# meilisearch/arroy

Measured on AMD Instinct MI355X. Metric: distances/sec, Q=1 batched 768-dim cosine scan (GB/s vs HBM roofline in `roofline`); tree-build seconds at 10M vectors in `build_10m`, higher is better.
Workload: dtype f32; 1 GPU; 1M x 768 cosine Q=1 scan (configs[1])

## Files before the change

arroy_amd/csrc/common.h:

```cpp
#pragma once

#include <hip/hip_runtime.h>

#include <algorithm>
#include <cstdarg>
#include <cstdint>
#include <cstdio>
#include <atomic>
#include <cstring>
#include <mutex>
#include <new>
#include <string>
#include <thread>
#include <vector>

#include "../../include/arroy_hip.h"
#include "../../include/arroy_hip_policy.h"

namespace ah {

void set_error(const char *fmt, ...);
const char *last_error();
void set_error_status(int status);
void set_error_detail(uint32_t item, uint64_t expected, uint64_t received);
// ... 102 lines not shown
    X(PAIR_GROUP, "AH_PAIR_GROUP", 0)                                                                                    \
    X(PAIR_RUNS, "AH_PAIR_RUNS", 1)                                                                                      \
    X(SEARCH_BITMAP, "AH_SEARCH_BITMAP", 1)          \
    X(SEARCH_TILES, "AH_SEARCH_TILES", 1)                          \
    X(SEARCH_WAVE, "AH_SEARCH_WAVE", 1)                        \
    X(SEARCH_BLOCK_MAX_QUERIES, "AH_SEARCH_BLOCK_MAX_QUERIES", 64)  \
    X(SEARCH_SMALL_GATE, "AH_SEARCH_SMALL_GATE", 1)  \
    X(SEARCH_SMALL_UNITS_MAX_QUERIES, "AH_SEARCH_SMALL_UNITS_MAX_QUERIES", 64)  \
    X(SEARCH_FUSED_FLAG, "AH_SEARCH_FUSED_FLAG", 1)  \
    X(SEARCH_FUSED_PREPARE, "AH_SEARCH_FUSED_PREPARE", 1)  \
    X(SEARCH_SINGLE_FUSED, "AH_SEARCH_SINGLE_FUSED", 1)  \
    X(SEARCH_SMALL_TILES_MAX_QUERIES, "AH_SEARCH_SMALL_TILES_MAX_QUERIES", 8)  \
    X(SEARCH_MULTI, "AH_SEARCH_MULTI", 1)        \
    X(SEARCH_MULTI_TREES_PER_BLOCK, "AH_SEARCH_MULTI_TREES_PER_BLOCK", 8)  \
    X(SEARCH_MULTI_IDS_BY_TILES, "AH_SEARCH_MULTI_IDS_BY_TILES", 1)  \
    X(SEARCH_SPIN_WAIT, "AH_SEARCH_SPIN_WAIT", 1)  \
    X(SEARCH_FLAT_TILES, "AH_SEARCH_FLAT_TILES", 1)  \
    X(SEARCH_STATUS_WIPE, "AH_SEARCH_STATUS_WIPE", 1)  \
    X(SEARCH_ITEM_LIST, "AH_SEARCH_ITEM_LIST", 1)  \
    X(SEARCH_MULTI_OWN_UNITS, "AH_SEARCH_MULTI_OWN_UNITS", 1)  \
    X(SEARCH_MULTI_TRACE, "AH_SEARCH_MULTI_TRACE", 0)  \
    X(SEARCH_MULTI_MAX_QUERIES, "AH_SEARCH_MULTI_MAX_QUERIES", 32)  \
    X(EXACT_WIDE, "AH_EXACT_WIDE", 1)            \
    X(RERANK_GROUPS, "AH_RERANK_GROUPS", 2)      \
    X(RERANK_SCREEN8, "AH_RERANK_SCREEN8", 1)    \
    X(SEARCH_SCREEN8_MAX_VISITS, "AH_SEARCH_SCREEN8_MAX_VISITS", 4)  \
    X(SEARCH_SCREEN8_MIN_QUERIES, "AH_SEARCH_SCREEN8_MIN_QUERIES", 65)  \
    X(SEARCH_SCREEN8, "AH_SEARCH_SCREEN8", 1)    \
    X(RERANK_SCREEN, "AH_RERANK_SCREEN", 1)      \
    X(REPLICATE_HOST_BOUNCE, "AH_REPLICATE_HOST_BOUNCE", 0)  \
    X(RERANK_TIMING, "AH_RERANK_TIMING", 0)      \
    X(SEARCH_SCREEN, "AH_SEARCH_SCREEN", 1)      \
    X(SEARCH_FILTER_GROUP_MIN, "AH_SEARCH_FILTER_GROUP_MIN", 16)  \
    X(FILTER_COMBINE_SHORTCUT, "AH_FILTER_COMBINE_SHORTCUT", 1)  \
    X(AUDIT_COVER_MB, "AH_AUDIT_COVER_MB", 64)  \
    X(HOST_THREADS, "AH_HOST_THREADS", 8)             \
    X(DEVICE_CACHE_MB, "AH_DEVICE_CACHE_MB", 98304)  \
    X(HOST_CACHE_MB, "AH_HOST_CACHE_MB", 16384)    \
    X(CACHE_KEEP_IDLE, "AH_CACHE_KEEP_IDLE", 0)  \
    X(FAIL_ALLOC_AFTER, "AH_FAIL_ALLOC_AFTER", 0)  \
    X(STAGE_THREADS, "AH_STAGE_THREADS", 0)                                                                              \
    X(STAGE_MEMCPY, "AH_STAGE_MEMCPY", 0)                                                                                \
    X(STAGE_REGISTER, "AH_STAGE_REGISTER", 0)
enum Tunable {
#define AH_X(id, name, def) TUN_##id,
    AH_TUNABLES(AH_X)
// ... 340 lines not shown
```

arroy_amd/csrc/dense_device.h:

```cpp
#pragma once

namespace ah {

typedef _Float16 f16x8_t __attribute__((ext_vector_type(8)));
typedef float f32x16_t __attribute__((ext_vector_type(16)));
typedef float f32x4_t __attribute__((ext_vector_type(4)));

constexpr uint32_t kDM = 256;
template <int WN>
struct DenseShape {
    static constexpr uint32_t kBN = 64u * WN;
    static constexpr uint32_t kThreads = 128u * WN;
    static constexpr uint32_t kWaves = 2u * WN;
    static constexpr uint32_t kStage = (kDM + kBN) * 128u;
    static constexpr uint32_t kPiecesA = 32u / kWaves, kPiecesB = (kBN / 8u) / kWaves;
};
constexpr uint32_t kDenseHalf = 128;
constexpr uint32_t kDensePitch = kDM + 4;
constexpr uint32_t kDenseLds = kDenseHalf * kDensePitch * 4;
constexpr uint32_t kDenseGroup = 8;
static_assert(2 * DenseShape<4>::kStage <= kDenseLds && 2 * DenseShape<2>::kStage <= kDenseLds, "stage buffers fit");

constexpr uint32_t kSideUndecided = 2u;
constexpr uint32_t kSideVerify = 4u;

struct DenseArgs {
    const uint16_t *rows;
    const float4 *stats;
    const float *headers;
    uint64_t n;
    uint32_t hpitch;
    const uint8_t *shadow;
    uint64_t hstride;
    uint32_t n_cols;
    const FNode *nodes;
    const uint32_t *node_of;
    uint8_t *side_bytes;
    float gamma_s, gamma_r;
    uint32_t n_row_tiles, n_col_tiles, group, verify;
};

template <int WN>
__device__ __forceinline__ void dense_stage(const uint8_t *const (&a_src)[DenseShape<WN>::kPiecesA],
                                            const uint8_t *const (&b_src)[DenseShape<WN>::kPiecesB], uint32_t kb, uint8_t *stage,
                                            uint32_t wave) {
    typedef DenseShape<WN> SH;
    const uint64_t koff = (uint64_t)kb * 128u;
// ... 450 lines not shown
```

arroy_amd/csrc/forest.hip:

```cpp
#include <algorithm>
#include <atomic>
#include <chrono>
#include <condition_variable>
#include <deque>
#include <thread>
#include <cstdlib>
#include <immintrin.h>
#include <sys/mman.h>
#include <sys/syscall.h>
#include <unistd.h>
#include <new>

#include "common.h"
#include "split_device.h"
#include "screen_device.h"

namespace ah {

static constexpr uint32_t kTile = 2048;
static constexpr int kBlock = 256;
static constexpr int kMaxBlocks = 4096;

enum { ST_PENDING = 0, ST_ACCEPTED = 1, ST_RANDOM = 2 };

// ... 1044 lines not shown
        if (threadIdx.x == 0) {
            tile_left[tile] = s_left;
            if (s_left) atomicAdd(&nodes[tl.node].n_left, s_left);
        }
    }
    __syncthreads();
    if (threadIdx.x == 0) s_fb = s_bad = s_n8 = s_d8 = s_d8b = 0;
    __syncthreads();
    if (j == 0 && fallbacks) atomicAdd(&s_fb, fallbacks);
    if (j == 0 && bad) atomicAdd(&s_bad, bad);
    if (j == 0 && met8) atomicAdd(&s_n8, met8);
    if (j == 0 && decided8) atomicAdd(&s_d8, decided8);
    if (j == 0 && decided8b) atomicAdd(&s_d8b, decided8b);
    __syncthreads();
    if (threadIdx.x == 0) {
        if (s_fb) atomicAdd(&counters->fallbacks, (unsigned long long)s_fb);
        if (s_bad) atomicAdd(&counters->violations, (unsigned long long)s_bad);
        if (s_n8) atomicAdd(&counters->stage8_pairs, (unsigned long long)s_n8);
        if (s_d8) atomicAdd(&counters->stage8_decided, (unsigned long long)s_d8);
        if (s_d8b) atomicAdd(&counters->stage8b_decided, (unsigned long long)s_d8b);
    }
}

template <int METRIC>
__device__ __forceinline__ float rows_exact_margin(const DataView &dv, uint64_t row, const uint8_t *nrec, uint64_t hdr_off,
                                                   uint32_t j) {
    const float *rp = dv.rows_f32 + row * dv.pitch;
    const float *np = reinterpret_cast<const float *>(nrec);
    const float d = octet_reduce_stream<OP_DOT>(reinterpret_cast<const float4 *>(np), rp, dv.dims, j);
    const float *nh = reinterpret_cast<const float *>(nrec + hdr_off);
    if (METRIC == AH_EUCLIDEAN || METRIC == AH_MANHATTAN) return f_add(nh[0], d);
    if (METRIC == AH_DOT_PRODUCT) return f_add(d, f_mul(nh[0], dv.headers[2 * row]));
    return d;
}

template <int METRIC>
__device__ __forceinline__ float rows_exact_margin_wide(const DataView &dv, uint64_t row, const uint8_t *nrec, uint64_t hdr_off,
                                                        uint32_t j) {
    const float *rp = dv.rows_f32 + row * dv.pitch;
    const float *np = reinterpret_cast<const float *>(nrec);
    const float *nh = reinterpret_cast<const float *>(nrec + hdr_off);
    float h0 = 0.0f, rh = 0.0f;
    if (METRIC == AH_EUCLIDEAN || METRIC == AH_MANHATTAN || METRIC == AH_DOT_PRODUCT) h0 = nh[0];
    if (METRIC == AH_DOT_PRODUCT) rh = dv.headers[2 * row];
    const float d = octet_reduce_wide<OP_DOT, false>(np, rp, dv.dims, j);
    if (METRIC == AH_EUCLIDEAN || METRIC == AH_MANHATTAN) return f_add(h0, d);
// ... 50 lines not shown
        const uint32_t rem = slot % per_chunk;
        tile = rem % sch.tiles;
        group = ((x + 8u - (chunk & 7u)) & 7u) + 8u * (rem / sch.tiles);
        if (group >= sch.n_groups) return false;
    } else {
        const uint32_t per_chunk = sch.n_groups * sch.tiles;
        chunk = sch.chunk0 + b / per_chunk;
        const uint32_t in_chunk = b % per_chunk;
        group = in_chunk / sch.tiles;
        tile = in_chunk % sch.tiles;
    }
    row_begin = (uint64_t)chunk * sch.chunk_rows + (uint64_t)tile * sch.rows_per_block;
    row_end = min(min(row_begin + sch.rows_per_block, (uint64_t)(chunk + 1) * sch.chunk_rows), n_rows);
    return row_begin < row_end;
}
__global__ void k_rows_schedule_coverage(RowsSchedule sch, uint64_t n_rows, uint32_t *__restrict__ counts) {
    uint32_t group;
    uint64_t row_begin, row_end;
    if (!rows_block_map(sch, blockIdx.x, n_rows, group, row_begin, row_end)) return;
    for (uint64_t row = row_begin + (threadIdx.x >> 3); row < row_end; row += blockDim.x >> 3)
        if ((threadIdx.x & 7u) == 0) atomicAdd(&counts[(uint64_t)group * n_rows + row], 1u);
}

template <int METRIC, int TC, bool LDS_NORMALS>
__global__ __launch_bounds__(LDS_NORMALS ? (TC >= 16 ? 512 : 1024) : kBlock,
                             LDS_NORMALS ? 1 : (AH_SCREEN_WAVES > 1 ? AH_SCREEN_WAVES : (TC == 8 ? 4 : 1))) void k_forest_screen_rows(
    DataView dv, ScreenView sv, const uint32_t *__restrict__ node_of, uint32_t tree_base, uint32_t n_pass,
    const uint8_t *__restrict__ normals, uint64_t nstride, uint64_t hdr_off, const uint8_t *__restrict__ shadow,
    uint64_t hstride, uint8_t *__restrict__ side_bytes, RowsSchedule sch, const AbortFlags abort_flag,
    ScreenCounters *__restrict__ counters, uint32_t verify) {
    extern __shared__ uint4 s_shadow4[];
    __shared__ uint32_t s_fb, s_bad;
    if (abort_requested(abort_flag)) return;
    uint32_t group;
    uint64_t row_begin, row_end;
    if (!rows_block_map(sch, blockIdx.x, dv.n, group, row_begin, row_end)) return;
    const uint32_t tree0 = tree_base + group * TC;
    const uint32_t hstride4 = (uint32_t)(hstride >> 4);
    uint32_t first_node = 0;
    if (LDS_NORMALS) {
        first_node = sch.tree_first[tree0];
        const uint32_t n_group_nodes = sch.tree_first[tree0 + n_pass] - first_node;
        const uint4 *g = reinterpret_cast<const uint4 *>(shadow + (uint64_t)first_node * hstride);
        const uint32_t total = n_group_nodes * hstride4;
        for (uint32_t i = threadIdx.x; i < total; i += blockDim.x) s_shadow4[i] = g[i];
    }
    if (threadIdx.x == 0) s_fb = s_bad = 0;
    __syncthreads();
    const uint32_t j = threadIdx.x & 7u;
    const uint32_t octets = blockDim.x >> 3;
    const uint32_t steps = sv.hpitch >> 6;
    const uint32_t stats4 = sv.hpitch >> 3;
    const uint4 *base4 = LDS_NORMALS ? s_shadow4 : reinterpret_cast<const uint4 *>(shadow);
    const uint32_t node0 = first_node;
    const uint32_t last_tree = n_pass - 1;
    constexpr int N = TC >= 8 ? 8 : TC;
    constexpr int SETS = TC >= 8 ? TC / 8 : 1;
    const uint32_t my_t = octet_owned_tree<N>(j);
    const bool owner = octet_is_owner<N>(j);
    uint32_t fallbacks = 0, bad = 0;
    for (uint64_t row = row_begin + (threadIdx.x >> 3); row < row_end; row += octets) {
        const uint4 *r4 = reinterpret_cast<const uint4 *>(sv.rows + row * sv.hpitch) + j;
        uint32_t my_node[SETS];
        uint32_t noff[TC];
        float acc[TC];
#pragma unroll
        for (int st = 0; st < SETS; st++)
            my_node[st] = node_of[(uint64_t)(tree0 + min(my_t + 8u * st, last_tree)) * dv.n + row];
#pragma unroll
        for (int t = 0; t < TC; t++) {
// ... 13 lines not shown
        for (; k < steps; k++) {
            const uint4 x = r4[k * 8];
#pragma unroll
            for (int t = 0; t < TC; t++) acc[t] = screen_dot8(base4[noff[t] + k * 8], x, acc[t]);
        }
        const float4 rs = sv.stats[row];
        const float row_extra = METRIC == AH_DOT_PRODUCT ? dv.headers[2 * row] : 0.0f;
#pragma unroll
        for (int st = 0; st < SETS; st++) {
            const float total = octet_transpose_sum<N>(acc + 8 * st, j);
            const uint32_t t = my_t + 8u * st;
            const bool valid = owner && t <= last_tree && my_node[st] != 0xFFFFFFFFu;
            uint32_t side = 0;
            bool decided = false;
            if (valid) {
                const uint4 raw = base4[(my_node[st] - node0) * hstride4 + stats4];
                NormalStats ns;
                ns.an = __uint_as_float(raw.x);
                ns.bn = __uint_as_float(raw.y);
                ns.cn = __uint_as_float(raw.z);
                ns.extra = __uint_as_float(raw.w);
                decided = screen_decides<METRIC>(total, rs, ns, row_extra, sv.gamma_s, sv.gamma_r, side);
            }
            const unsigned long long und = __ballot(valid && (!decided || verify));
            const uint32_t mask8 = (uint32_t)(und >> (8u * ((threadIdx.x & 63u) >> 3))) & 0xFFu;
            if (mask8) {
#pragma unroll
                for (int tt = 0; tt < N; tt++) {
                    constexpr uint32_t kOwner[8] = {octet_owner_lane<N>(0), octet_owner_lane<N>(1), octet_owner_lane<N>(2),
                                                    octet_owner_lane<N>(3), octet_owner_lane<N>(4), octet_owner_lane<N>(5),
                                                    octet_owner_lane<N>(6), octet_owner_lane<N>(7)};
                    const uint32_t ol = kOwner[tt];
                    if ((mask8 >> ol) & 1u) {
                        const uint32_t node = (noff[8 * st + tt] - j) / hstride4 + node0;
                        const uint32_t exact =
                            side_of_margin(rows_exact_margin<METRIC>(dv, row, normals + (uint64_t)node * nstride, hdr_off, j));
                        if (j == ol) {
                            if (decided && exact != side) bad++;
                            if (!decided) fallbacks++;
                            side = exact;
                        }
                    }
                }
            }
            if (valid) side_bytes[(uint64_t)(tree0 + t) * dv.n + row] = (uint8_t)side;
        }
    }
    if (fallbacks) atomicAdd(&s_fb, fallbacks);
    if (bad) atomicAdd(&s_bad, bad);
    __syncthreads();
    if (threadIdx.x == 0) {
        if (s_fb) atomicAdd(&counters->fallbacks, (unsigned long long)s_fb);
        if (s_bad) atomicAdd(&counters->violations, (unsigned long long)s_bad);
    }
}

struct NextCounts {
    uint32_t kids, tiles;
};
__device__ __forceinline__ void child_counts(const FNode &nd, uint32_t split_after, uint32_t cnt[2], uint32_t split[2]) {
    cnt[0] = nd.n_left;
    cnt[1] = nd.count - nd.n_left;
    split[0] = cnt[0] > split_after ? 1u : 0u;
    split[1] = cnt[1] > split_after ? 1u : 0u;
}
__global__ __launch_bounds__(256) void k_next_count(const FNode *__restrict__ nodes, uint32_t n_nodes, uint32_t split_after,
                                                    NextCounts *__restrict__ block_sums) {
    __shared__ uint32_t s_k[4], s_t[4];
    const uint32_t i = blockIdx.x * 256 + threadIdx.x;
    uint32_t kids = 0, tiles = 0;
// ... 421 lines not shown
        AH_HIP(create_copy_stream(&side));
        return AH_OK;
    }
    ~BatchCleanup() {
        if (side) (void)hipStreamSynchronize(side);
        for (hipEvent_t e : ev_attempt)
            if (e) (void)hipEventDestroy(e);
        for (hipEvent_t e : {ev_begin, ev_end, ev_level, ev_copy[0], ev_copy[1]})
            if (e) (void)hipEventDestroy(e);
        if (side) (void)hipStreamDestroy(side);
    }
};

struct CostPt {
    double mb, ns;
};
template <size_t N>
double interp(const CostPt (&t)[N], double mb) {
    if (mb <= t[0].mb) return t[0].ns;
    for (size_t i = 1; i < N; i++)
        if (mb <= t[i].mb) return t[i - 1].ns + (t[i].ns - t[i - 1].ns) * (mb - t[i - 1].mb) / (t[i].mb - t[i - 1].mb);
    return t[N - 1].ns;
}
double rows_pass_ns_per_row(uint32_t tc, double ws_mb, bool screened) {
    static const CostPt e16[] = {{0.4, 1.60}, {3.2, 1.83}, {6.3, 2.05}, {12.6, 2.33}, {25, 5.08}, {50, 6.05}, {100, 6.5}, {400, 6.8}};
    static const CostPt e8[] = {{0.2, 1.16}, {1.6, 1.22}, {3.2, 2.0}, {6.3, 2.5}, {12.6, 3.1}, {25, 3.5}, {100, 3.7}};
    static const CostPt e4[] = {{0.1, 0.73}, {0.8, 0.85}, {3.2, 0.88}, {6.3, 1.07}, {12.6, 1.45}, {25, 1.85}, {50, 2.05}, {100, 2.14}};
    static const CostPt e2[] = {{0.05, 0.49}, {0.8, 0.60}, {3.1, 0.62}, {6.3, 0.74}, {12.6, 0.99}, {25, 1.14}, {50, 1.21}};
    static const CostPt s16[] = {{0.025, 1.11}, {0.2, 1.13}, {0.4, 1.20}, {0.8, 1.25}, {1.6, 1.30}, {3.2, 1.45}, {6.4, 1.99},
                                 {12.7, 2.94}, {25, 3.57}, {51, 3.92}, {102, 4.10}, {203, 4.21}};
    static const CostPt s8[] = {{0.012, 0.58}, {0.1, 0.61}, {0.2, 0.67}, {0.4, 0.71}, {0.8, 0.74}, {1.6, 0.77}, {3.2, 0.85},
                                {6.4, 1.24}, {12.7, 1.66}, {25, 1.94}, {51, 2.09}, {102, 2.15}};
    static const CostPt s4[] = {{0.025, 0.325}, {0.05, 0.353}, {0.1, 0.415}, {0.2, 0.463}, {0.4, 0.493}, {0.8, 0.511},
                                {1.7, 0.45}, {3.4, 0.50}, {6.8, 0.69}, {13.6, 0.90}, {27, 1.03}, {54, 1.10}};
    static const CostPt s2[] = {{0.003, 0.235}, {0.05, 0.243}, {0.1, 0.261}, {0.2, 0.274}, {0.4, 0.284}, {0.8, 0.292},
                                {1.6, 0.314}, {3.2, 0.389}, {6.4, 0.49}, {12.7, 0.56}, {25, 0.60}};
    if (screened) return tc >= 16 ? interp(s16, ws_mb) : tc == 8 ? interp(s8, ws_mb) : tc == 4 ? interp(s4, ws_mb) : interp(s2, ws_mb);
    return tc >= 16 ? interp(e16, ws_mb) : tc == 8 ? interp(e8, ws_mb) : tc == 4 ? interp(e4, ws_mb) : interp(e2, ws_mb);
}

enum { MM_NODE = 0, MM_ROWS2 = 1, MM_ROWS4 = 2, MM_ROWS8 = 3, MM_ROWS16 = 4, MM_LDS8 = 5, MM_LDS16 = 6, MM_BQ = 7 };
inline int mm_rows(uint32_t tc) { return tc >= 16 ? MM_ROWS16 : tc == 8 ? MM_ROWS8 : tc == 4 ? MM_ROWS4 : MM_ROWS2; }

}

static size_t records_pool_trim() {
    RecordsPool &pool = records_pool();
    std::vector<HostRec> r;
    std::vector<uint32_t> i;
    {
        std::lock_guard<std::mutex> lk(pool.mu);
        r.swap(pool.recs);
        i.swap(pool.index);
    }
    return r.capacity() * sizeof(HostRec) + i.capacity() * sizeof(uint32_t);
}
static uint64_t normal_record_stride(const ah_dataset *ds) {
    const uint64_t raw = ds->row_bytes() + 16;
    return metric_is_bq(ds->metric) ? raw : (raw + 127) & ~(uint64_t)127;
// ... 381 lines not shown
            std::lock_guard<std::mutex> lk(mu);
            stop = true;
        }
        cv.notify_all();
        th.join();
    }
};

namespace {
struct ScreenRowsArgs {
    DataView dv;
    ScreenView sv;
    const uint32_t *node_of;
    uint32_t tree_base, n_pass;
    const uint8_t *normals;
    uint64_t nstride, hdr_off;
    const uint8_t *shadow;
    uint64_t hstride;
    uint8_t *side_bytes;
    RowsSchedule sch;
    AbortFlags abort_flag;
    ScreenCounters *counters;
    uint32_t verify;
};
template <int M, int TC, bool LDS>
int launch_screen_rows_inst(const ScreenRowsArgs &a, unsigned grid, size_t sh, hipStream_t s, int device) {
    const unsigned threads = LDS ? (TC >= 16 ? 512u : 1024u) : (unsigned)kBlock;
    if (LDS) {
        static std::atomic<bool> opt_in[64];
        if (!opt_in[device & 63].load(std::memory_order_acquire)) {
            AH_HIP(hipFuncSetAttribute(reinterpret_cast<const void *>(k_forest_screen_rows<M, TC, LDS>),
                                       hipFuncAttributeMaxDynamicSharedMemorySize, (int)kLdsNormalsBytes));
            opt_in[device & 63].store(true, std::memory_order_release);
        }
    }
    hipLaunchKernelGGL((k_forest_screen_rows<M, TC, LDS>), dim3(grid), dim3(threads), LDS ? sh : 0, s, a.dv, a.sv, a.node_of,
                       a.tree_base, a.n_pass, a.normals, a.nstride, a.hdr_off, a.shadow, a.hstride, a.side_bytes, a.sch,
                       a.abort_flag, a.counters, a.verify);
    return AH_OK;
}
template <int M>
int launch_screen_rows_metric(uint32_t tc, bool lds, const ScreenRowsArgs &a, unsigned grid, size_t sh, hipStream_t s, int device) {
    if (lds) return tc >= 16 ? launch_screen_rows_inst<M, 16, true>(a, grid, sh, s, device)
                             : launch_screen_rows_inst<M, 8, true>(a, grid, sh, s, device);
    switch (tc) {
    case 16: return launch_screen_rows_inst<M, 16, false>(a, grid, sh, s, device);
    case 8: return launch_screen_rows_inst<M, 8, false>(a, grid, sh, s, device);
    case 4: return launch_screen_rows_inst<M, 4, false>(a, grid, sh, s, device);
    default: return launch_screen_rows_inst<M, 2, false>(a, grid, sh, s, device);
    }
}
int launch_screen_rows(int metric, uint32_t tc, bool lds, const ScreenRowsArgs &a, unsigned grid, size_t sh, hipStream_t s,
                       int device) {
    switch (metric) {
    case AH_EUCLIDEAN: return launch_screen_rows_metric<AH_EUCLIDEAN>(tc, lds, a, grid, sh, s, device);
    case AH_MANHATTAN: return launch_screen_rows_metric<AH_MANHATTAN>(tc, lds, a, grid, sh, s, device);
    case AH_COSINE: return launch_screen_rows_metric<AH_COSINE>(tc, lds, a, grid, sh, s, device);
    default: return launch_screen_rows_metric<AH_DOT_PRODUCT>(tc, lds, a, grid, sh, s, device);
    }
}
}

namespace {
struct DensePlan {
    uint32_t n_row_tiles, n_col_tiles, group;
    bool wide;
    int narrow;
    bool stream;
    uint32_t tile_rows, tile_cols, threads, lds;
    uint64_t grid;
};
DensePlan dense_plan(uint64_t N, uint32_t n_cols) {
    DensePlan p{};
// ... 81 lines not shown
};

static int build_batch(ah_dataset *ds, const ah_build_options *opt, uint32_t first_tree, uint32_t n_trees,
                       uint32_t split_after, ah_forest *forest, Context *ctx, const uint32_t *subset_ids,
                       const uint64_t *subset_offsets, StreamBuild *sb = nullptr) {
    const uint64_t N = ds->n;
    const auto t_batch = std::chrono::steady_clock::now();
    std::vector<uint64_t> tree_base(n_trees + 1, 0);
    for (uint32_t t = 0; t < n_trees; t++)
        tree_base[t + 1] = tree_base[t] + (subset_ids ? subset_offsets[first_tree + t + 1] - subset_offsets[first_tree + t] : N);
    const uint64_t M = tree_base[n_trees];
    const DataView dv = ds->view();
    hipStream_t s = ctx->stream;
    const bool bq = metric_is_bq(ds->metric);
    const uint64_t hdr_off = ds->row_bytes();
    const uint64_t nstride = normal_record_stride(ds);
    const bool g_screen = tun(TUN_SCREEN) != 0, g_screen_verify = tun(TUN_SCREEN_VERIFY) != 0;
    const int g_rows_force = (int)tun(TUN_ROWMAJOR), g_dense = (int)tun(TUN_DENSE);
    const uint32_t g_tile_blocks = (uint32_t)std::max<long long>(1, tun(TUN_FOREST_TILE_BLOCKS));
    const uint32_t g_node_blocks = (uint32_t)std::max<long long>(0, tun(TUN_FOREST_NODE_BLOCKS));
    const uint32_t g_split_blocks = (uint32_t)std::max<long long>(1, tun(TUN_FOREST_SPLIT_BLOCKS));
    const uint32_t g_row_blocks = (uint32_t)std::max<long long>(1, tun(TUN_FOREST_ROW_BLOCKS));
    const bool g_rows_advance = tun(TUN_ROWMAJOR_ADVANCE) != 0, g_rows_lds = tun(TUN_ROWMAJOR_LDS) != 0;
    const uint32_t g_rows_max_tc = (uint32_t)std::max<long long>(2, tun(TUN_ROWMAJOR_MAX_TC));
    const double g_rows_cache_mb = (double)tun(TUN_ROWMAJOR_CACHE_MB);
    const uint32_t g_dense_max_cols = (uint32_t)std::max<long long>(0, tun(TUN_DENSE_MAX_COLS));
    const double g_dense_gmacs = (double)std::max<long long>(1, tun(TUN_DENSE_GMACS));
    const int timing = (int)tun(TUN_TIMING);
    const bool g_retry_gate = tun(TUN_RETRY_GATE) != 0;
    const uint32_t env_mode = (uint32_t)tun(TUN_MARGIN_MODE) & 0xFFFu;
    const uint32_t mode_req = (opt->margin_mode & 0xFFFu) ? (opt->margin_mode & 0xFFFu) : env_mode;
    const bool exact_only = (opt->margin_mode & AH_MARGIN_EXACT_ONLY) != 0 || !g_screen;

    const uint64_t max_nodes = M / ((uint64_t)split_after + 1) + n_trees;
    const uint64_t max_tiles = M / kTile + n_trees + max_nodes;
    DevBuf<uint32_t> perm_a, perm_b, final_perm, tile_left, tile_left_off, d_child, d_small;
    DevBuf<FNode> d_nodes_a, d_nodes_b, d_nodes_c;
    DevBuf<GroupInfo> d_groups;
    DevBuf<FTile> d_tiles;
    DevBuf<uint64_t> masks;
    DevBuf<NextCounts> d_block_sums;
    AH_TRY(perm_a.ensure(M));
    AH_TRY(perm_b.ensure(M));
    AH_TRY(final_perm.ensure(M));
    AH_TRY(d_nodes_a.ensure(max_nodes));
    AH_TRY(d_nodes_b.ensure(max_nodes));
// ... 612 lines not shown
                                                 : std::min<uint32_t>(n_tiles, std::max<uint32_t>(2048u, std::min<uint32_t>(65536u, n_tiles / 16u)));
        const unsigned masks_grid = n_nodes <= 4 * n_trees ? std::min<uint32_t>(tile_grid, 32768u) : tile_grid;

        const uint64_t rec_bytes = screen ? hstride : nstride;
        const uint64_t nodes_per_tree = (n_nodes + n_trees - 1) / n_trees;
        uint32_t row_tc = 0, lds_tc = 0, lds_worst = 0;
        double best_cost = -1.0;
        if (grouped) {
        } else if (rows_allowed && mode_req == AH_MARGIN_AUTO) {
            const double scale = screen ? (double)ds->hpitch * 2 / 1536.0 : (double)ds->row_bytes() / 3072.0;
            const double node8_ns = sv.rows8_lo ? std::min(0.24, 0.135 + 0.15 * ds->screen8_quality)
                                                : std::min(0.24, 0.155 + 0.125 * ds->screen8_quality);
            const double node_ns = screen ? (screen8 && ds->metric != AH_DOT_PRODUCT ? node8_ns : 0.24) : 0.47;
            const double active = (double)info.pairs / ((double)n_trees * (double)N);
            const double cost_node = (double)info.pairs * node_ns * scale;
            const double convert = (double)n_trees * (double)N *
                                   ((prev_rows && g_rows_advance ? 0.007 : 0.01 + 0.03 * std::min(1.0, (double)nodes_per_tree / 256.0)) +
                                    0.012 * std::min(1.0, (double)nodes_per_tree / 512.0));
            double best = 0.97 * cost_node;
            const double floor_ns = screen ? 0.15 : 0.45;
            auto launch_ns_per_row = [&](uint32_t tcv, uint32_t groups) {
                double ws_mb = (double)((uint64_t)tcv * nodes_per_tree * rec_bytes) / 1e6;
                if (groups <= 2 && tcv >= 16) ws_mb *= 0.5;
                return groups * (floor_ns + (rows_pass_ns_per_row(tcv, ws_mb, screen) - floor_ns) * std::min(1.0, active * 1.05));
            };
            for (uint32_t tc = std::min(16u, g_rows_max_tc); tc >= 2; tc >>= 1) {
                if (tc > 2 && tc / 2 >= n_trees) continue;
                const double ws_mb = (double)((uint64_t)tc * nodes_per_tree * rec_bytes) / 1e6;
                if (g_rows_cache_mb > 0 && ws_mb > g_rows_cache_mb) continue;
                double ns_per_row = n_trees / tc ? launch_ns_per_row(tc, n_trees / tc) : 0.0;
                for (uint32_t t0 = n_trees / tc * tc; t0 < n_trees;) {
                    const uint32_t rem = n_trees - t0;
                    uint32_t tcv = tc;
                    while (tcv > 2 && tcv > rem) tcv >>= 1;
                    for (uint32_t up = tcv << 1; up <= tc && tcv < rem; up <<= 1)
                        if (up >= rem && up - rem <= (up >= 16 ? 3u : 1u)) tcv = up;
                    ns_per_row += launch_ns_per_row(tcv, 1);
                    t0 += std::min(tcv, rem);
                }
                const double cost_rows = (double)N * ns_per_row * scale + convert;
                if (cost_rows < best || (g_rows_force == 1 && row_tc == 0)) {
                    best = std::min(best, cost_rows);
                    row_tc = tc;
                }
            }
            best_cost = best;
        } else if (rows_allowed && mode_req != AH_MARGIN_DENSE_MFMA) {
            row_tc = mode_req & 0xFFu;
        }
        bool dense = false;
        const DensePlan dp_legal = dense_plan(N, std::max(n_nodes, 1u));
        const bool dense_legal = !grouped && rows_allowed && screen && g_dense != 0 && n_nodes <= g_dense_max_cols &&
                                 (dp_legal.grid + 64) * (uint64_t)dp_legal.threads < 0xFFFFFFFFull && dp_legal.grid < 0x7FFFFFFFull;
        if (dense_legal && mode_req == AH_MARGIN_DENSE_MFMA) {
            dense = true;
        } else if (dense_legal && mode_req == AH_MARGIN_AUTO) {
            const uint32_t bn = n_nodes > 128 ? 256u : 128u;
            const double cols = (double)(((uint64_t)n_nodes + bn - 1) / bn * bn);
            const double hscale = (double)ds->hpitch / 768.0;
            const double per_row = std::max(std::max(0.40 * hscale, 0.25), 0.17 * hscale + 0.0023 * n_trees + cols * (double)ds->hpitch / g_dense_gmacs);
            const double convert = (double)n_trees * (double)N * (prev_rows && g_rows_advance ? 0.007 : 0.04);
            const double cost_dense = (double)N * per_row + (double)info.pairs * (0.002 + 0.006 * (double)ds->row_bytes() / 3072.0) + convert;
            dense = g_dense == 1 || best_cost < 0 || cost_dense < best_cost;
// ... 56 lines not shown
            AH_SPLIT_KERNEL(AH_SPLIT_LAUNCH)
#undef AH_SPLIT_LAUNCH
            AH_DBG(s, "create_split");
            if (screen)
                hipLaunchKernelGGL(k_forest_shadow_normals, dim3(std::min<uint32_t>(n_nodes, attempt ? 65536u : 1u << 20)), dim3(64), 0, s,
                                   dv, d_cur, chunk_d, nstride, hdr_off, shadow_d, hstride, sv.hpitch, n_nodes, gate);
            if (screen8 && !(attempt == 0 && row_tc >= 2))
                hipLaunchKernelGGL(k_forest_shadow_normals8, dim3(std::min<uint32_t>(n_nodes, 65536u)), dim3(64), 0, s, dv, d_cur,
                                   n_nodes, chunk_d, nstride, hdr_off, ds->d_dim_scale, shadow8_d, stride8, sv.pitch8, gate);
            AH_HIP(hipEventRecord(bc.ev_attempt[2 * attempt], s));
            if (attempt == 0 && row_tc >= 2) {
                if (prev_rows && g_rows_advance) {
                    hipLaunchKernelGGL(k_forest_advance_node_of, dim3(kMaxBlocks), dim3(kBlock), 0, s, node_of.p, side_bytes.p,
                                       d_child.p, (uint64_t)n_trees * N);
                    if (info.n_fix)
                        hipLaunchKernelGGL(k_forest_assign_node_of, dim3(std::min<uint32_t>(n_tiles, kMaxBlocks)), dim3(kBlock), 0,
                                           s, d_cur, d_tiles.p, n_tiles, cur, N, node_of.p, 1u);
                } else {
                    AH_HIP(hipMemsetAsync(node_of.p, 0xFF, (size_t)n_trees * N * 4, s));
                    hipLaunchKernelGGL(k_forest_assign_node_of, dim3(tile_grid), dim3(kBlock), 0, s, d_cur, d_tiles.p, n_tiles,
                                       cur, N, node_of.p, 0u);
                }
                uint32_t passes = 0;
                if (dense) {
                    DenseArgs da{};
                    da.rows = sv.rows;
                    da.stats = sv.stats;
                    da.headers = dv.headers;
                    da.n = N;
                    da.hpitch = sv.hpitch;
                    da.shadow = shadow_d;
                    da.hstride = hstride;
                    da.n_cols = n_nodes;
                    da.nodes = d_cur;
                    da.node_of = node_of.p;
                    da.side_bytes = side_bytes.p;
                    da.gamma_s = (float)(2.0 * ((double)sv.hpitch + (double)sv.hpitch / 16 + 16.0) * 1.1920929e-7);
                    da.gamma_r = sv.gamma_r;
                    const DensePlan dp = dense_plan(N, n_nodes);
                    da.n_row_tiles = dp.n_row_tiles;
                    da.n_col_tiles = dp.n_col_tiles;
                    da.group = dp.group;
                    da.verify = verify;
                    const bool wide = dp.wide;
                    const uint64_t dgrid = dp.grid;
                    AH_REQUIRE(dgrid < 0x7FFFFFFFull, AH_ERR_INVALID_ARGUMENT, "forest build: too many tiles for one launch");
                    const unsigned egrid = exact_pairs_grid(N, n_trees);
#define AH_DENSE_WN(M, WNV)                                                                                              \
    do {                                                                                                                 \
        static std::atomic<bool> dense_opt_in[64];                               \
        if (!dense_opt_in[ds->device & 63].load(std::memory_order_acquire)) {                                            \
            AH_HIP(hipFuncSetAttribute(reinterpret_cast<const void *>(k_forest_dense_screen<M, WNV>),                    \
                                       hipFuncAttributeMaxDynamicSharedMemorySize, (int)kDenseLds));                     \
            dense_opt_in[ds->device & 63].store(true, std::memory_order_release);                                        \
        }                                                                                                                \
        hipLaunchKernelGGL((k_forest_dense_screen<M, WNV>), dim3((unsigned)dgrid), dim3(DenseShape<WNV>::kThreads),      \
                           kDenseLds, s, da, d_abort);                                                                   \
    } while (0)
#define AH_DENSE_NARROW(M, NTV)                                                                                          \
    do {                                                                                                                 \
        if (dp.stream)                                                                                                   \
            hipLaunchKernelGGL((k_forest_dense_narrow<M, NTV, true>), dim3((unsigned)dgrid), dim3(kNarrowThreads),       \
                               NarrowShape<NTV>::kLds, s, da, d_abort);                                                  \
        else                                                                                                             \
            hipLaunchKernelGGL((k_forest_dense_narrow<M, NTV, false>), dim3((unsigned)dgrid), dim3(kNarrowThreads),      \
                               NarrowShape<NTV>::kLds, s, da, d_abort);                                                  \
    } while (0)
#define AH_DENSE(M)                                                                                                      \
    do {                                                                                                                 \
        if (dp.narrow == 2) AH_DENSE_NARROW(M, 2);                                                                       \
        else if (dp.narrow == 4) AH_DENSE_NARROW(M, 4);                                                                  \
        else if (wide) AH_DENSE_WN(M, 4);                                                                                \
        else AH_DENSE_WN(M, 2);                                                                                          \
        if (tun(TUN_EXACT_WIDE) != 0)                                                                                    \
            hipLaunchKernelGGL((k_forest_exact_pairs<M, true>), dim3(egrid), dim3(256), 0, s, dv, node_of.p, side_bytes.p, \
                               n_trees, chunk_d, nstride, hdr_off, d_counters, d_abort);                                 \
        else                                                                                                             \
            hipLaunchKernelGGL((k_forest_exact_pairs<M>), dim3(egrid), dim3(256), 0, s, dv, node_of.p, side_bytes.p,     \
                               n_trees, chunk_d, nstride, hdr_off, d_counters, d_abort);                                 \
    } while (0)
                    switch (ds->metric) {
                    case AH_EUCLIDEAN: AH_DENSE(AH_EUCLIDEAN); break;
                    case AH_MANHATTAN: AH_DENSE(AH_MANHATTAN); break;
                    case AH_COSINE: AH_DENSE(AH_COSINE); break;
                    default: AH_DENSE(AH_DOT_PRODUCT); break;
                    }
#undef AH_DENSE_WN
#undef AH_DENSE_NARROW
#undef AH_DENSE
                    forest->stats.dense_launches++;
                    forest->stats.dense_columns += n_nodes;
                    passes = 1;
                } else if (screen) {
                    const uint32_t gtc = lds_tc ? lds_tc : row_tc;
                    ScreenRowsArgs ra{dv, sv, node_of.p, 0, 0, chunk_d, nstride, hdr_off, shadow_d, hstride, side_bytes.p,
                                      RowsSchedule{}, d_abort, d_counters, verify};
                    if (lds_tc) {
                        memcpy(h_tree_first, tree_first.data(), ((size_t)n_trees + 1) * 4);
                        AH_HIP(hipMemcpyAsync(d_tree_first_fixed, h_tree_first, ((size_t)n_trees + 1) * 4, hipMemcpyHostToDevice, s));
                    }
                    const size_t lds_sh = (size_t)lds_worst * rec_bytes;
                    auto launch = [&](uint32_t tcv, uint32_t t0, uint32_t groups, uint32_t np) -> int {
                        RowsPlan plan;
                        AH_TRY(plan_rows_launches(N, sv.hpitch, tcv, groups, lds_tc != 0, (uint64_t)tcv * nodes_per_tree * rec_bytes, &plan));
                        ra.tree_base = t0;
                        ra.n_pass = np;
                        ra.sch = plan.sch;
                        ra.sch.tree_first = d_tree_first_fixed;
                        for (const auto &l : plan.launches) {
                            ra.sch.chunk0 = l.first;
                            AH_TRY(launch_screen_rows(ds->metric, tcv, lds_tc != 0, ra, l.second, lds_sh, s, ds->device));
                        }
                        forest->stats.margin_mode_launches[lds_tc ? (tcv >= 16 ? MM_LDS16 : MM_LDS8) : mm_rows(tcv)]++;
                        forest->stats.rows_xcd_launches += plan.xcd ? plan.launches.size() : 0;
                        forest->stats.rows_nt_launches += plan.nt ? plan.launches.size() : 0;
                        forest->stats.rows_split_launches += plan.launches.size() - 1;
                        passes += groups;
                        return AH_OK;
                    };
                    const uint32_t full = n_trees / gtc;
                    if (full) AH_TRY(launch(gtc, 0, full, gtc));
                    for (uint32_t t0 = full * gtc; t0 < n_trees;) {
                        const uint32_t rem = n_trees - t0;
                        uint32_t tcv = gtc;
                        if (!lds_tc) {
                            while (tcv > 2 && tcv > rem) tcv >>= 1;
                            for (uint32_t up = tcv << 1; up <= gtc && tcv < rem; up <<= 1)
                                if (up >= rem && up - rem <= (up >= 16 ? 3u : 1u)) tcv = up;
                        }
                        const uint32_t np = std::min<uint32_t>(tcv, rem);
                        AH_TRY(launch(tcv, t0, 1, np));
                        t0 += np;
                    }
                }
                const unsigned row_grid = (unsigned)std::min<uint64_t>((N + 31) / 32, g_row_blocks);
                for (uint32_t t0 = 0; t0 < n_trees && lds_tc && !screen; t0 += lds_tc) {
                    const uint32_t np = std::min<uint32_t>(lds_tc, n_trees - t0);
                    const uint32_t first = tree_first[t0], cnt = tree_first[t0 + np] - first;
                    if (cnt == 0) continue;
                    const size_t sh = (size_t)cnt * rec_bytes;
                    const unsigned per_cu = (unsigned)std::max<size_t>(1, std::min<size_t>(2, (150u << 10) / std::max<size_t>(sh, 1)));
                    const unsigned lthreads = lds_tc >= 16 ? 512u : 1024u;
                    const unsigned lgrid = (unsigned)std::min<uint64_t>((N * 8 + lthreads - 1) / lthreads, 256u * per_cu);
#define AH_LDS_OPT_IN(KERNEL)                                                                                          \
    do {                                                                                                               \
        static std::atomic<bool> lds_opt_in[64];                                \
        if (!lds_opt_in[ds->device & 63].load(std::memory_order_acquire)) {                                            \
            AH_HIP(hipFuncSetAttribute(reinterpret_cast<const void *>(KERNEL), hipFuncAttributeMaxDynamicSharedMemorySize, \
                                       (int)kLdsNormalsBytes));                                                        \
            lds_opt_in[ds->device & 63].store(true, std::memory_order_release);                                        \
        }                                                                                                              \
    } while (0)
#define AH_ROWS_LDS(M, TCV)                                                                                              \
    do {                                                                                                                 \
        AH_LDS_OPT_IN((k_forest_margin_rows_lds<M, TCV>));                                                               \
        hipLaunchKernelGGL((k_forest_margin_rows_lds<M, TCV>), dim3(lgrid), dim3(lthreads), sh, s, dv, node_of.p, t0, np,  \
// ... 857 lines not shown
```

Measured before the change: 3.051 billion distances/s.

## Defer exact margin fallbacks in screened row kernel to separate exact-pairs pass

The screened row-major forest kernel gains a DEFER variant that only writes undecided/verify markers into side bytes and skips the inline exact-dot fallback. A separate k_forest_exact_pairs launch, shared with the dense path, then resolves those pairs. The goal is to stop divergent per-octet exact work from stalling the screening loop. The cost model gets new deferred-pass tables plus an exact-pairs cost term, so the tree-count choice can shift, and there is one extra kernel launch.

```diff
diff --git a/arroy_amd/csrc/common.h b/arroy_amd/csrc/common.h
--- a/arroy_amd/csrc/common.h
+++ b/arroy_amd/csrc/common.h
@@ -148,6 +148,7 @@
     X(SEARCH_MULTI_TRACE, "AH_SEARCH_MULTI_TRACE", 0)  \
     X(SEARCH_MULTI_MAX_QUERIES, "AH_SEARCH_MULTI_MAX_QUERIES", 32)  \
     X(EXACT_WIDE, "AH_EXACT_WIDE", 1)            \
+    X(ROWS_DEFER_EXACT, "AH_ROWS_DEFER_EXACT", 1)  \
     X(RERANK_GROUPS, "AH_RERANK_GROUPS", 2)      \
     X(RERANK_SCREEN8, "AH_RERANK_SCREEN8", 1)    \
     X(SEARCH_SCREEN8_MAX_VISITS, "AH_SEARCH_SCREEN8_MAX_VISITS", 4)  \
diff --git a/arroy_amd/csrc/dense_device.h b/arroy_amd/csrc/dense_device.h
--- a/arroy_amd/csrc/dense_device.h
+++ b/arroy_amd/csrc/dense_device.h
@@ -21,8 +21,6 @@
 constexpr uint32_t kDenseGroup = 8;
 static_assert(2 * DenseShape<4>::kStage <= kDenseLds && 2 * DenseShape<2>::kStage <= kDenseLds, "stage buffers fit");
 
-constexpr uint32_t kSideUndecided = 2u;
-constexpr uint32_t kSideVerify = 4u;
 
 struct DenseArgs {
     const uint16_t *rows;
diff --git a/arroy_amd/csrc/forest.hip b/arroy_amd/csrc/forest.hip
--- a/arroy_amd/csrc/forest.hip
+++ b/arroy_amd/csrc/forest.hip
@@ -1090,6 +1090,9 @@
     }
 }
 
+constexpr uint32_t kSideUndecided = 2u;
+constexpr uint32_t kSideVerify = 4u;
+
 template <int METRIC>
 __device__ __forceinline__ float rows_exact_margin(const DataView &dv, uint64_t row, const uint8_t *nrec, uint64_t hdr_off,
                                                    uint32_t j) {
@@ -1186,7 +1189,7 @@
         if ((threadIdx.x & 7u) == 0) atomicAdd(&counts[(uint64_t)group * n_rows + row], 1u);
 }
 
-template <int METRIC, int TC, bool LDS_NORMALS>
+template <int METRIC, int TC, bool LDS_NORMALS, bool DEFER>
 __global__ __launch_bounds__(LDS_NORMALS ? (TC >= 16 ? 512 : 1024) : kBlock,
                              LDS_NORMALS ? 1 : (AH_SCREEN_WAVES > 1 ? AH_SCREEN_WAVES : (TC == 8 ? 4 : 1))) void k_forest_screen_rows(
     DataView dv, ScreenView sv, const uint32_t *__restrict__ node_of, uint32_t tree_base, uint32_t n_pass,
@@ -1209,7 +1212,7 @@
         const uint32_t total = n_group_nodes * hstride4;
         for (uint32_t i = threadIdx.x; i < total; i += blockDim.x) s_shadow4[i] = g[i];
     }
-    if (threadIdx.x == 0) s_fb = s_bad = 0;
+    if (!DEFER && threadIdx.x == 0) s_fb = s_bad = 0;
     __syncthreads();
     const uint32_t j = threadIdx.x & 7u;
     const uint32_t octets = blockDim.x >> 3;
@@ -1269,6 +1272,12 @@
                 ns.extra = __uint_as_float(raw.w);
                 decided = screen_decides<METRIC>(total, rs, ns, row_extra, sv.gamma_s, sv.gamma_r, side);
             }
+            if (DEFER) {
+                if (valid)
+                    side_bytes[(uint64_t)(tree0 + t) * dv.n + row] =
+                        (uint8_t)(decided ? (verify ? (kSideVerify | side) : side) : kSideUndecided);
+                continue;
+            }
             const unsigned long long und = __ballot(valid && (!decided || verify));
             const uint32_t mask8 = (uint32_t)(und >> (8u * ((threadIdx.x & 63u) >> 3))) & 0xFFu;
             if (mask8) {
@@ -1293,6 +1302,7 @@
             if (valid) side_bytes[(uint64_t)(tree0 + t) * dv.n + row] = (uint8_t)side;
         }
     }
+    if (DEFER) return;
     if (fallbacks) atomicAdd(&s_fb, fallbacks);
     if (bad) atomicAdd(&s_bad, bad);
     __syncthreads();
@@ -1760,7 +1770,7 @@
         if (mb <= t[i].mb) return t[i - 1].ns + (t[i].ns - t[i - 1].ns) * (mb - t[i - 1].mb) / (t[i].mb - t[i - 1].mb);
     return t[N - 1].ns;
 }
-double rows_pass_ns_per_row(uint32_t tc, double ws_mb, bool screened) {
+double rows_pass_ns_per_row(uint32_t tc, double ws_mb, bool screened, bool deferred = false) {
     static const CostPt e16[] = {{0.4, 1.60}, {3.2, 1.83}, {6.3, 2.05}, {12.6, 2.33}, {25, 5.08}, {50, 6.05}, {100, 6.5}, {400, 6.8}};
     static const CostPt e8[] = {{0.2, 1.16}, {1.6, 1.22}, {3.2, 2.0}, {6.3, 2.5}, {12.6, 3.1}, {25, 3.5}, {100, 3.7}};
     static const CostPt e4[] = {{0.1, 0.73}, {0.8, 0.85}, {3.2, 0.88}, {6.3, 1.07}, {12.6, 1.45}, {25, 1.85}, {50, 2.05}, {100, 2.14}};
@@ -1773,6 +1783,16 @@
                                 {1.7, 0.45}, {3.4, 0.50}, {6.8, 0.69}, {13.6, 0.90}, {27, 1.03}, {54, 1.10}};
     static const CostPt s2[] = {{0.003, 0.235}, {0.05, 0.243}, {0.1, 0.261}, {0.2, 0.274}, {0.4, 0.284}, {0.8, 0.292},
                                 {1.6, 0.314}, {3.2, 0.389}, {6.4, 0.49}, {12.7, 0.56}, {25, 0.60}};
+    static const CostPt d16[] = {{0.025, 0.743}, {0.2, 0.762}, {0.4, 0.840}, {0.8, 0.896}, {1.6, 0.990}, {3.2, 1.174}, {6.4, 1.293},
+                                 {12.7, 1.876}, {25, 3.053}, {51, 3.665}, {102, 3.961}, {203, 4.106}};
+    static const CostPt d8[] = {{0.012, 0.387}, {0.1, 0.421}, {0.2, 0.484}, {0.4, 0.526}, {0.8, 0.572}, {1.6, 0.614}, {3.2, 0.711},
+                                {6.4, 0.988}, {12.7, 1.491}, {25, 1.774}, {51, 1.987}, {102, 2.083}};
+    static const CostPt d4[] = {{0.025, 0.227}, {0.05, 0.263}, {0.1, 0.329}, {0.2, 0.378}, {0.4, 0.408}, {0.8, 0.422},
+                                {1.7, 0.372}, {3.4, 0.461}, {6.8, 0.644}, {13.6, 0.871}, {27, 1.001}, {54, 1.073}};
+    static const CostPt d2[] = {{0.003, 0.191}, {0.05, 0.204}, {0.1, 0.224}, {0.2, 0.239}, {0.4, 0.249}, {0.8, 0.256},
+                                {1.6, 0.283}, {3.2, 0.366}, {6.4, 0.467}, {12.7, 0.544}, {25, 0.587}};
+    if (screened && deferred)
+        return tc >= 16 ? interp(d16, ws_mb) : tc == 8 ? interp(d8, ws_mb) : tc == 4 ? interp(d4, ws_mb) : interp(d2, ws_mb);
     if (screened) return tc >= 16 ? interp(s16, ws_mb) : tc == 8 ? interp(s8, ws_mb) : tc == 4 ? interp(s4, ws_mb) : interp(s2, ws_mb);
     return tc >= 16 ? interp(e16, ws_mb) : tc == 8 ? interp(e8, ws_mb) : tc == 4 ? interp(e4, ws_mb) : interp(e2, ws_mb);
 }
@@ -2200,33 +2220,39 @@
     AbortFlags abort_flag;
     ScreenCounters *counters;
     uint32_t verify;
+    bool defer;
 };
-template <int M, int TC, bool LDS>
+template <int M, int TC, bool LDS, bool DEFER>
 int launch_screen_rows_inst(const ScreenRowsArgs &a, unsigned grid, size_t sh, hipStream_t s, int device) {
     const unsigned threads = LDS ? (TC >= 16 ? 512u : 1024u) : (unsigned)kBlock;
     if (LDS) {
         static std::atomic<bool> opt_in[64];
         if (!opt_in[device & 63].load(std::memory_order_acquire)) {
-            AH_HIP(hipFuncSetAttribute(reinterpret_cast<const void *>(k_forest_screen_rows<M, TC, LDS>),
+            AH_HIP(hipFuncSetAttribute(reinterpret_cast<const void *>(k_forest_screen_rows<M, TC, LDS, DEFER>),
                                        hipFuncAttributeMaxDynamicSharedMemorySize, (int)kLdsNormalsBytes));
             opt_in[device & 63].store(true, std::memory_order_release);
         }
     }
-    hipLaunchKernelGGL((k_forest_screen_rows<M, TC, LDS>), dim3(grid), dim3(threads), LDS ? sh : 0, s, a.dv, a.sv, a.node_of,
-                       a.tree_base, a.n_pass, a.normals, a.nstride, a.hdr_off, a.shadow, a.hstride, a.side_bytes, a.sch,
-                       a.abort_flag, a.counters, a.verify);
+    hipLaunchKernelGGL((k_forest_screen_rows<M, TC, LDS, DEFER>), dim3(grid), dim3(threads), LDS ? sh : 0, s, a.dv, a.sv,
+                       a.node_of, a.tree_base, a.n_pass, a.normals, a.nstride, a.hdr_off, a.shadow, a.hstride, a.side_bytes,
+                       a.sch, a.abort_flag, a.counters, a.verify);
     return AH_OK;
+}
+template <int M, bool DEFER>
+int launch_screen_rows_defer(uint32_t tc, bool lds, const ScreenRowsArgs &a, unsigned grid, size_t sh, hipStream_t s, int device) {
+    if (lds) return tc >= 16 ? launch_screen_rows_inst<M, 16, true, DEFER>(a, grid, sh, s, device)
+                             : launch_screen_rows_inst<M, 8, true, DEFER>(a, grid, sh, s, device);
+    switch (tc) {
+    case 16: return launch_screen_rows_inst<M, 16, false, DEFER>(a, grid, sh, s, device);
+    case 8: return launch_screen_rows_inst<M, 8, false, DEFER>(a, grid, sh, s, device);
+    case 4: return launch_screen_rows_inst<M, 4, false, DEFER>(a, grid, sh, s, device);
+    default: return launch_screen_rows_inst<M, 2, false, DEFER>(a, grid, sh, s, device);
+    }
 }
 template <int M>
 int launch_screen_rows_metric(uint32_t tc, bool lds, const ScreenRowsArgs &a, unsigned grid, size_t sh, hipStream_t s, int device) {
-    if (lds) return tc >= 16 ? launch_screen_rows_inst<M, 16, true>(a, grid, sh, s, device)
-                             : launch_screen_rows_inst<M, 8, true>(a, grid, sh, s, device);
-    switch (tc) {
-    case 16: return launch_screen_rows_inst<M, 16, false>(a, grid, sh, s, device);
-    case 8: return launch_screen_rows_inst<M, 8, false>(a, grid, sh, s, device);
-    case 4: return launch_screen_rows_inst<M, 4, false>(a, grid, sh, s, device);
-    default: return launch_screen_rows_inst<M, 2, false>(a, grid, sh, s, device);
-    }
+    return a.defer ? launch_screen_rows_defer<M, true>(tc, lds, a, grid, sh, s, device)
+                   : launch_screen_rows_defer<M, false>(tc, lds, a, grid, sh, s, device);
 }
 int launch_screen_rows(int metric, uint32_t tc, bool lds, const ScreenRowsArgs &a, unsigned grid, size_t sh, hipStream_t s,
                        int device) {
@@ -2354,6 +2380,7 @@
     const uint32_t g_split_blocks = (uint32_t)std::max<long long>(1, tun(TUN_FOREST_SPLIT_BLOCKS));
     const uint32_t g_row_blocks = (uint32_t)std::max<long long>(1, tun(TUN_FOREST_ROW_BLOCKS));
     const bool g_rows_advance = tun(TUN_ROWMAJOR_ADVANCE) != 0, g_rows_lds = tun(TUN_ROWMAJOR_LDS) != 0;
+    const bool g_rows_defer = tun(TUN_ROWS_DEFER_EXACT) != 0;
     const uint32_t g_rows_max_tc = (uint32_t)std::max<long long>(2, tun(TUN_ROWMAJOR_MAX_TC));
     const double g_rows_cache_mb = (double)tun(TUN_ROWMAJOR_CACHE_MB);
     const uint32_t g_dense_max_cols = (uint32_t)std::max<long long>(0, tun(TUN_DENSE_MAX_COLS));
@@ -3012,8 +3039,9 @@
             auto launch_ns_per_row = [&](uint32_t tcv, uint32_t groups) {
                 double ws_mb = (double)((uint64_t)tcv * nodes_per_tree * rec_bytes) / 1e6;
                 if (groups <= 2 && tcv >= 16) ws_mb *= 0.5;
-                return groups * (floor_ns + (rows_pass_ns_per_row(tcv, ws_mb, screen) - floor_ns) * std::min(1.0, active * 1.05));
+                return groups * (floor_ns + (rows_pass_ns_per_row(tcv, ws_mb, screen, g_rows_defer) - floor_ns) * std::min(1.0, active * 1.05));
             };
+            const double cost_exact = screen && g_rows_defer ? (double)info.pairs * (0.002 + 0.006 * (double)ds->row_bytes() / 3072.0) : 0.0;
             for (uint32_t tc = std::min(16u, g_rows_max_tc); tc >= 2; tc >>= 1) {
                 if (tc > 2 && tc / 2 >= n_trees) continue;
                 const double ws_mb = (double)((uint64_t)tc * nodes_per_tree * rec_bytes) / 1e6;
@@ -3028,7 +3056,7 @@
                     ns_per_row += launch_ns_per_row(tcv, 1);
                     t0 += std::min(tcv, rem);
                 }
-                const double cost_rows = (double)N * ns_per_row * scale + convert;
+                const double cost_rows = (double)N * ns_per_row * scale + convert + cost_exact;
                 if (cost_rows < best || (g_rows_force == 1 && row_tc == 0)) {
                     best = std::min(best, cost_rows);
                     row_tc = tc;
@@ -3131,6 +3159,25 @@
                                        cur, N, node_of.p, 0u);
                 }
                 uint32_t passes = 0;
+                auto launch_exact_pairs = [&]() {
+                    const unsigned egrid = exact_pairs_grid(N, n_trees);
+#define AH_EXACT(M)                                                                                                      \
+    do {                                                                                                                 \
+        if (tun(TUN_EXACT_WIDE) != 0)                                                                                    \
+            hipLaunchKernelGGL((k_forest_exact_pairs<M, true>), dim3(egrid), dim3(256), 0, s, dv, node_of.p, side_bytes.p, \
+                               n_trees, chunk_d, nstride, hdr_off, d_counters, d_abort);                                 \
+        else                                                                                                             \
+            hipLaunchKernelGGL((k_forest_exact_pairs<M>), dim3(egrid), dim3(256), 0, s, dv, node_of.p, side_bytes.p,     \
+                               n_trees, chunk_d, nstride, hdr_off, d_counters, d_abort);                                 \
+    } while (0)
+                    switch (ds->metric) {
+                    case AH_EUCLIDEAN: AH_EXACT(AH_EUCLIDEAN); break;
+                    case AH_MANHATTAN: AH_EXACT(AH_MANHATTAN); break;
+                    case AH_COSINE: AH_EXACT(AH_COSINE); break;
+                    default: AH_EXACT(AH_DOT_PRODUCT); break;
+                    }
+#undef AH_EXACT
+                };
                 if (dense) {
                     DenseArgs da{};
                     da.rows = sv.rows;
@@ -3154,7 +3201,6 @@
                     const bool wide = dp.wide;
                     const uint64_t dgrid = dp.grid;
                     AH_REQUIRE(dgrid < 0x7FFFFFFFull, AH_ERR_INVALID_ARGUMENT, "forest build: too many tiles for one launch");
-                    const unsigned egrid = exact_pairs_grid(N, n_trees);
 #define AH_DENSE_WN(M, WNV)                                                                                              \
     do {                                                                                                                 \
         static std::atomic<bool> dense_opt_in[64];                               \
@@ -3181,12 +3227,6 @@
         else if (dp.narrow == 4) AH_DENSE_NARROW(M, 4);                                                                  \
         else if (wide) AH_DENSE_WN(M, 4);                                                                                \
         else AH_DENSE_WN(M, 2);                                                                                          \
-        if (tun(TUN_EXACT_WIDE) != 0)                                                                                    \
-            hipLaunchKernelGGL((k_forest_exact_pairs<M, true>), dim3(egrid), dim3(256), 0, s, dv, node_of.p, side_bytes.p, \
-                               n_trees, chunk_d, nstride, hdr_off, d_counters, d_abort);                                 \
-        else                                                                                                             \
-            hipLaunchKernelGGL((k_forest_exact_pairs<M>), dim3(egrid), dim3(256), 0, s, dv, node_of.p, side_bytes.p,     \
-                               n_trees, chunk_d, nstride, hdr_off, d_counters, d_abort);                                 \
     } while (0)
                     switch (ds->metric) {
                     case AH_EUCLIDEAN: AH_DENSE(AH_EUCLIDEAN); break;
@@ -3197,13 +3237,14 @@
 #undef AH_DENSE_WN
 #undef AH_DENSE_NARROW
 #undef AH_DENSE
+                    launch_exact_pairs();
                     forest->stats.dense_launches++;
                     forest->stats.dense_columns += n_nodes;
                     passes = 1;
                 } else if (screen) {
                     const uint32_t gtc = lds_tc ? lds_tc : row_tc;
                     ScreenRowsArgs ra{dv, sv, node_of.p, 0, 0, chunk_d, nstride, hdr_off, shadow_d, hstride, side_bytes.p,
-                                      RowsSchedule{}, d_abort, d_counters, verify};
+                                      RowsSchedule{}, d_abort, d_counters, verify, g_rows_defer};
                     if (lds_tc) {
                         memcpy(h_tree_first, tree_first.data(), ((size_t)n_trees + 1) * 4);
                         AH_HIP(hipMemcpyAsync(d_tree_first_fixed, h_tree_first, ((size_t)n_trees + 1) * 4, hipMemcpyHostToDevice, s));
@@ -3241,6 +3282,7 @@
                         AH_TRY(launch(tcv, t0, 1, np));
                         t0 += np;
                     }
+                    if (g_rows_defer) launch_exact_pairs();
                 }
                 const unsigned row_grid = (unsigned)std::min<uint64_t>((N + 31) / 32, g_row_blocks);
                 for (uint32_t t0 = 0; t0 < n_trees && lds_tc && !screen; t0 += lds_tc) {
```

New measurement: 3.034 billion distances/s. Within noise of the previous version (-0.6%).
